# IBM/AdaMML

Measured on AMD Instinct MI355X. Metric: clips/sec (train fwd+bwd) RGB+Audio AdaMML @224^2, 5 seg, higher is better.
Workload: dtype bf16

## Files before the change

### adamml_amd/csrc/conv_gemm.hip

```cpp
#include "common.h"
#include "../../include/adamml_hip.h"
#include <type_traits>
#include <stdlib.h>
#include <stdio.h>


namespace {

constexpr int BP = 128;
constexpr int BK = 32;
constexpr int NTHREADS = 256;

struct ConvP {
    const bf16_t* x;
    const bf16_t* w;
    const float* in_scale;
    const float* in_shift;
    bf16_t* y;
    double* stats;
    int N, H, W, Cin, OH, OW, Cout, KH, KW, stride, pad, up, up_shift, act, accumulate;
    int P, K, cin_shift, n_ptiles, n_ctiles, tpb;
    size_t gx, gy;
    int in_gstride;
    const bf16_t* bn_z;
    const float* bn_vec;
    int bn_act;
    const bf16_t* res_out;
    const uint8_t* res_mask;
    int res_act;
    const bf16_t* bn_z2;
    const float* bn_vec2;
    double* stats2;
    const bf16_t* x2;
    const float* aff;
    bf16_t* side;
    const bf16_t* xb;
    int K1, C2;
    size_t gw;
    const float* epi_add;
    const float* id_scale;
    const float* id_shift;
    int id_gstride;
    uint8_t* mask_out;
    const bf16_t* pf_a;
    const float* pf_scale;
    const float* pf_shift;
    float* pf_ws;
    int pf_act, pf_gs, pf_nsplit;
    int wK;
    int cls_nt;
    unsigned cls_code;
    int oH, oW, o_ph, o_pw;
    int tp_nblk, tp_Q;
    bf16_t* tp_y;
    uint16_t* tp_code;
};

__device__ __forceinline__ int lds_off(int row, int chunk) {
    return row * 64 + ((chunk ^ (((row >> 3) & 1) << 1)) << 4);
}

template <int N, class F>
__device__ __forceinline__ void static_for(F&& f) {
    if constexpr (N > 0) {
        static_for<N - 1>(f);
        f(std::integral_constant<int, N - 1>{});
    }
}

template <int CH>
__device__ __forceinline__ int tr_swz(int row) {
    if (CH >= 128) return ((row & 3) | (((row >> 3) & 1) << 2)) << 2;
    return (((row >> 1) & 1) | (((row >> 3) & 1) << 1)) << 2;
}

__device__ const uint4 g_zero_page[4] = {};

__device__ __forceinline__ void glds16(const void* gsrc, unsigned lds_dst_uniform) {
    unsigned keep;
    asm volatile("s_mov_b32 %0, m0\n\ts_mov_b32 m0, %2\n\ts_nop 0\n\tglobal_load_lds_dwordx4 %1, off\n\ts_mov_b32 m0, %0"
                 : "=&s"(keep) : "v"(gsrc), "s"(lds_dst_uniform) : "memory");
}

constexpr int conv_gemm_wg_per_cu(int BC, int MODE, int PD, bool RES, bool DUAL, bool CAT, bool FADD, bool GLDS, int EID, int EPI) {
    if (RES || DUAL || CAT || EID) return 2;
    const int n = PD == 1 ? (BC == 128 ? 3 : 4) : (BC == 128 ? 2 : 3);
    const bool fewer = (MODE == 2 && !(BC == 128 && PD == 3)) || FADD ||
                       (BC == 64 && PD == 1 && ((EPI == 1 && !(MODE == 0 && GLDS)) || (EPI == 2 && MODE == 1))) ||
                       (BC == 128 && MODE == 1 && EPI == 2 && !GLDS);
    return fewer ? n - 1 : n;
}

template <int BC, int MODE, int PD, bool RES = false, bool DUAL = false, bool CAT = false, bool FADD = false, bool GLDS = false, int EID = 0,
          bool LZF = false, int EPI = -1, bool PF = false, int TP = 0>
__global__ __launch_bounds__(NTHREADS, conv_gemm_wg_per_cu(BC, MODE, PD, RES, DUAL, CAT, FADD, GLDS, EID, EPI)) void conv_gemm_kernel(ConvP p) {
    static_assert(TP == 0 || (FADD && EID && MODE == 0 && BC == 128 && (TP == 2 || TP == 4 || TP == 8)), "TP: FADD + EID, 128-wide cout tiles");
    constexpr int PPF = TP ? BP / TP : BP;
    constexpr int WCT = BC / 32;
    constexpr int WROWS = BC / 64;
    constexpr int TILE_BYTES = (BP + BC) * 64;
    constexpr int EPI_BYTES = BP * (BC * 2 + 16);
    constexpr int NBUF = GLDS ? 3 : 2;
    constexpr int STAGE_BYTES = (NBUF * TILE_BYTES) > EPI_BYTES ? (NBUF * TILE_BYTES) : EPI_BYTES;
    constexpr int NSR = (FADD || EPI == 0) ? 1 : 4;
    constexpr int CS_BYTES = NSR * 2 * BC * 4;
    constexpr int CS2_OFF = STAGE_BYTES + CS_BYTES + (MODE == 0 ? 0 : 256) + (MODE == 3 ? BP * 4 + 16 : 0);
    constexpr int VEC_MAXK = 1024;
    constexpr int VEC_OFF = CS2_OFF + (RES ? CS_BYTES : 0);
    constexpr int LZF_MAXK = 512;
    constexpr int PF_C = 64;
    constexpr int PF_OFF = (VEC_OFF + (LZF ? 2 * LZF_MAXK * 4 : (MODE == 0 && !GLDS) ? (DUAL ? 3 : 2) * VEC_MAXK * 4 : 0) + 1023) / 1024 * 1024;
    constexpr int SMEM_BYTES = PF ? PF_OFF + BP * PF_C * 2 : VEC_OFF + (LZF ? 2 * LZF_MAXK * 4 : (MODE == 0 && !GLDS) ? (DUAL ? 3 : 2) * VEC_MAXK * 4 : 0);
    __shared__ __attribute__((aligned(1024))) char smem[SMEM_BYTES];

    {
        const int g = blockIdx.y;
        p.x += (size_t)g * p.gx;
        p.y += (size_t)g * p.gy;
        if (p.stats) p.stats += (size_t)g * ADAMML_STAT_SLOTS * 2 * p.Cout;
        if (p.in_scale) { p.in_scale += (size_t)g * p.in_gstride; p.in_shift += (size_t)g * p.in_gstride; }
        if (p.bn_z) { p.bn_z += (size_t)g * p.gy; p.bn_vec += (size_t)g * 4 * p.Cout; }
        if (CAT) {
            p.xb += (size_t)g * (p.gx / p.K1) * p.C2;
            p.w += (size_t)g * p.gw;
            p.epi_add += (size_t)g * p.Cout;
        }
        if (DUAL) {
            p.x2 += (size_t)g * p.gx;
            p.aff += (size_t)g * 3 * p.K;
            if (p.side) p.side += (size_t)g * p.gx;
        }
        if (FADD) {
            p.bn_vec += (size_t)g * 4 * p.Cout;
            if (p.res_out) p.res_out += (size_t)g * p.gy;
            if (p.mask_out) p.mask_out += ((size_t)g * p.gy) >> 3;
            if (p.id_scale) { p.id_scale += (size_t)g * p.id_gstride; p.id_shift += (size_t)g * p.id_gstride; }
            if (TP) { p.tp_y += (size_t)g * (p.gy >> 1); if (p.tp_code) p.tp_code += ((size_t)g * (p.gy >> 1)) >> 3; }
        }
        if (PF) {
            p.pf_a += (size_t)g * p.P * PF_C;
            if (p.pf_scale) { p.pf_scale += (size_t)g * p.pf_gs; p.pf_shift += (size_t)g * p.pf_gs; }
        }
        if (RES) {
            p.res_out += (size_t)g * p.gy;
            if (p.res_mask) p.res_mask += ((size_t)g * p.gy) >> 3;
            if (p.bn_z2) { p.bn_z2 += (size_t)g * p.gy; p.bn_vec2 += (size_t)g * 4 * p.Cout; p.stats2 += (size_t)g * ADAMML_STAT_SLOTS * 2 * p.Cout; }
        }
    }
    const int tid = threadIdx.x;
    float* s_vec = reinterpret_cast<float*>(smem + (MODE == 0 ? VEC_OFF : 0));
    const int nvec = CAT ? p.C2 : p.K;
    const bool vec_lds = MODE == 0 && nvec <= VEC_MAXK && (DUAL || p.in_scale != nullptr);
    if (LZF) {
        const int kpad = (p.K + BK - 1) / BK * BK;
        for (int i = tid; i < kpad; i += NTHREADS) {
            s_vec[i] = i < p.K ? p.in_scale[i] : 0.f;
            s_vec[LZF_MAXK + i] = i < p.K ? p.in_shift[i] : 0.f;
        }
        __syncthreads();
    } else
    if (vec_lds) {
        if (DUAL) {
            for (int i = tid; i < 3 * p.K; i += NTHREADS) s_vec[i] = p.aff[i];
        } else {
            for (int i = tid; i < nvec; i += NTHREADS) { s_vec[i] = p.in_scale[i]; s_vec[nvec + i] = p.in_shift[i]; }
        }
        __syncthreads();
    }
    const int lane = tid & 63;
    const int wave = tid >> 6;
    const int wp = wave & 1;
    const int wc = wave >> 1;

    const int nwg = gridDim.x;
    int bid = blockIdx.x;
    {
        const int q = nwg >> 3, r = nwg & 7, xcd = bid & 7, idx = bid >> 3;
        bid = (xcd < r ? xcd * (q + 1) : r * (q + 1) + (xcd - r) * q) + idx;
    }
    const int ctile = bid % p.n_ctiles;
    const int pgrp = bid / p.n_ctiles;
    const int c0 = ctile * BC;

    const int chunk = tid & 3;
    const int row_a = tid >> 2;
// ... 283 lines not shown
#pragma unroll
        for (int r = 0; r < WROWS; ++r) {
            bf16x8 v = rw[SL][r];
            if (UNC && !(w_ok[r] && rkok[UNC ? SL : 0])) v = bf16x8{0, 0, 0, 0, 0, 0, 0, 0};
            *reinterpret_cast<bf16x8*>(base + BP * 64 + lds_off(row_a + r * 64, chunk)) = v;
        }
    };

    f32x4 acc[WCT][4];
#pragma unroll
    for (int i = 0; i < WCT; ++i)
#pragma unroll
        for (int j = 0; j < 4; ++j) acc[i][j] = f32x4{0.f, 0.f, 0.f, 0.f};

    const int nk = (p.K + BK - 1) / BK;
    const bool tail_rows = TP ? tp_q0 + PPF > p.tp_Q : p0 + BP > p.P;
    auto compute = [&](int buf, int kt = 0) {
        const char* base = smem + buf * TILE_BYTES;
        bf16x8 fa[4], fw[WCT];
#pragma unroll
        for (int t = 0; t < 4; ++t)
            fa[t] = *reinterpret_cast<const bf16x8*>(base + lds_off(wp * 64 + t * 16 + li, lg));
        if constexpr (LZF) {
            const f32x8 sc = load_f32x8(s_vec + kt * BK + lg * 8), sh = load_f32x8(s_vec + LZF_MAXK + kt * BK + lg * 8);
            const float lo = act_lo(p.act), hi = act_hi(p.act);
#pragma unroll
            for (int t = 0; t < 4; ++t) {
                f32x8 f = bf8_to_f32(fa[t]);
#pragma unroll
                for (int i = 0; i < 8; ++i) f[i] = clamp_act(fmaf(f[i], sc[i], sh[i]), lo, hi);
                fa[t] = f32_to_bf8(f);
            }
            if (tail_rows) {
#pragma unroll
                for (int t = 0; t < 4; ++t) {
                    const int r = wp * 64 + t * 16 + li;
                    if (TP ? tp_q0 + (r % PPF) >= p.tp_Q : p0 + r >= p.P) fa[t] = bf16x8{0, 0, 0, 0, 0, 0, 0, 0};
                }
            }
        }
#pragma unroll
        for (int t = 0; t < WCT; ++t)
            fw[t] = *reinterpret_cast<const bf16x8*>(base + BP * 64 + lds_off(wc * (BC / 2) + t * 16 + li, lg));
#pragma unroll
        for (int ct = 0; ct < WCT; ++ct)
#pragma unroll
            for (int pt = 0; pt < 4; ++pt)
                acc[ct][pt] = __builtin_amdgcn_mfma_f32_16x16x32_bf16(fw[ct], fa[pt], acc[ct][pt], 0, 0, 0);
    };
    if constexpr (GLDS) {
        const bf16_t* zeros = reinterpret_cast<const bf16_t*>(g_zero_page);
        const unsigned lds0 = (unsigned)(size_t)(__attribute__((address_space(3))) char*)smem + wave * 1024;
        const int kc8 = (chunk ^ (((row_a >> 3) & 1) << 1)) * 8;
        auto glds_stage = [&](int kt, int buf) {
            const int k = kt * BK + kc8;
            const bool kok = k < p.K;
            const unsigned base = lds0 + buf * TILE_BYTES;
            int kw_off = k;
            if (MODE == 0) {
#pragma unroll
                for (int r = 0; r < 2; ++r) {
                    const bf16_t* src = (a_ok[r] && kok) ? p.x + (size_t)(unsigned)(a_base[r] + k) : zeros;
                    glds16(src, __builtin_amdgcn_readfirstlane(base + r * 4096));
                }
            } else {
                const int tap = kok ? (k >> p.cin_shift) : 0;
                const int ci = k & (p.Cin - 1);
                const int toff = s_tapoff[tap] + ci;
                if (MODE == 3) kw_off = s_wtap[tap] + ci;
#pragma unroll
                for (int r = 0; r < 2; ++r) {
                    const bool ok = kok && ((a_mask[r] >> tap) & 1ull);
                    const bf16_t* src = ok ? p.x + (size_t)(unsigned)(a_base[r] + toff) : zeros;
                    glds16(src, __builtin_amdgcn_readfirstlane(base + r * 4096));
                }
            }
#pragma unroll
            for (int r = 0; r < WROWS; ++r) {
                const bf16_t* src = (w_ok[r] && kok) ? wrow[r] + kw_off : zeros;
                glds16(src, __builtin_amdgcn_readfirstlane(base + BP * 64 + r * 4096));
            }
        };
        constexpr int PER = 2 + WROWS;
        glds_stage(0, 0);
        if (nk > 1) glds_stage(1, 1);
        issue_eid();
        int buf = 0;
        for (int kt = 0; kt < nk; ++kt) {
            if (NEID && kt <= 1) {
                if (kt + 1 < nk) asm volatile("s_waitcnt vmcnt(%0)" ::"n"(PER + NEID) : "memory");
                else asm volatile("s_waitcnt vmcnt(%0)" ::"n"(NEID) : "memory");
            } else
            if (kt + 1 < nk) asm volatile("s_waitcnt vmcnt(%0)" ::"n"(PER) : "memory");
            else asm volatile("s_waitcnt vmcnt(0)" ::: "memory");
            __builtin_amdgcn_s_barrier();
            if (kt + 2 < nk) glds_stage(kt + 2, buf == 0 ? 2 : buf - 1);
            compute(buf, kt);
            buf = buf == 2 ? 0 : buf + 1;
        }
    } else {
    int kt0 = 0;
    if (UNC && nk >= 2 * PD) {
        static_for<PD>([&](auto sc) { issue_loads(sc, (int)decltype(sc)::value); });
        for (; kt0 + 2 * PD <= nk; kt0 += PD) {
            static_for<PD>([&](auto sc) {
                const int kt = kt0 + (int)decltype(sc)::value;
                store_tile(sc, kt & 1);
                issue_loads(sc, kt + PD);
                __syncthreads();
                compute(kt & 1);
            });
        }
    } else {
    static_for<PD>([&](auto sc) {
        if ((int)decltype(sc)::value < nk) issue_loads(sc, (int)decltype(sc)::value);
    });
    }
    issue_eid();
    for (; kt0 < nk; kt0 += PD) {
        static_for<PD>([&](auto sc) {
            const int kt = kt0 + (int)decltype(sc)::value;
            if (kt < nk) {
                store_tile(sc, kt & 1);
                if (kt + PD < nk) issue_loads(sc, kt + PD);
                __syncthreads();
                compute(kt & 1);
            }
        });
    }
    }
    __syncthreads();

    f32x8 esum, esq, esq2;
#pragma unroll
    for (int i = 0; i < 8; ++i) esum[i] = esq[i] = esq2[i] = 0.f;
#pragma unroll
    for (int pt = 0; pt < 4; ++pt)
#pragma unroll
        for (int ct = 0; ct < WCT; ++ct) {
            const int prow = wp * 64 + pt * 16 + li;
            const int ccol = wc * (BC / 2) + ct * 16 + lg * 4;
            *reinterpret_cast<bf16x4*>(smem + prow * CROW + ccol * 2) = f32_to_bf4(acc[ct][pt]);
        }
    __syncthreads();
    if (FADD) {
        if (eco < p.Cout) {
            const f32x8 sc = load_f32x8(p.bn_vec + eco), sh = load_f32x8(p.bn_vec + p.Cout + eco);
            f32x8 isc, ish;
#pragma unroll
            for (int i = 0; i < 8; ++i) { isc[i] = 1.f; ish[i] = 0.f; }
            if (p.id_scale) { isc = load_f32x8(p.id_scale + eco); ish = load_f32x8(p.id_shift + eco); }
            const float rlo = act_lo(p.res_act), rhi = act_hi(p.res_act);
            constexpr int NR = BP / RSTEP, EB = EID ? NR : (NR < 4 ? NR : 4);
            if constexpr (TP != 0) {
                static_assert(RSTEP == 16 && NR == 8, "TP epilogue mapping");
                constexpr int NPX = PPF / 16, To = TP / 2;
                bf16x8 vb[NR];
#pragma unroll
                for (int j = 0; j < NR; ++j) {
                    const int r = erow0 + j * RSTEP;
                    f32x8 f = bf8_to_f32(*reinterpret_cast<const bf16x8*>(smem + r * CROW + ech * 16));
                    const f32x8 w = bf8_to_f32(eid[j]);
#pragma unroll
                    for (int i = 0; i < 8; ++i) f[i] = clamp_act(fmaf(f[i], sc[i], sh[i]) + fmaf(w[i], isc[i], ish[i]), rlo, rhi);
                    vb[j] = f32_to_bf8(f);
                }
#pragma unroll
                for (int s = 0; s < NPX; ++s) {
                    const int q = tp_q0 + erow0 + 16 * s;
                    if (q >= p.tp_Q) continue;
#pragma unroll
                    for (int to = 0; to < To; ++to) {
                        f32x8 best;
                        unsigned code = 0;
#pragma unroll
                        for (int i = 0; i < 8; ++i) best[i] = -INFINITY;
#pragma unroll
                        for (int k = 0; k < 3; ++k) {
                            const int tt = 2 * to - 1 + k;
                            if (tt < 0 || tt >= TP) continue;
                            const f32x8 v = bf8_to_f32(vb[tt * NPX + s]);
// ... 873 lines not shown
        for (; s + 48 < nsplit; s += 64) {
            a += *reinterpret_cast<const f32x4*>(ws + (size_t)s * n + i);
            a1 += *reinterpret_cast<const f32x4*>(ws + (size_t)(s + 16) * n + i);
            a2 += *reinterpret_cast<const f32x4*>(ws + (size_t)(s + 32) * n + i);
            a3 += *reinterpret_cast<const f32x4*>(ws + (size_t)(s + 48) * n + i);
        }
        for (; s < nsplit; s += 16) a += *reinterpret_cast<const f32x4*>(ws + (size_t)s * n + i);
        a = (a + a1) + (a2 + a3);
    }
    red[ty][tx] = a;
    __syncthreads();
    if (ty == 0 && i < n) {
        f32x4 t = {0.f, 0.f, 0.f, 0.f};
#pragma unroll
        for (int k = 0; k < 16; ++k) t += red[k][tx];
        if (taps > 1) {
            const size_t per_co = (size_t)taps * cin;
#pragma unroll
            for (int q = 0; q < 4; ++q) {
                const size_t ii = i + q;
                const size_t co = ii / per_co;
                const int rem = (int)(ii - co * per_co), tap = rem / cin, ci = rem - tap * cin;
                const size_t o = (co * cin + ci) * taps + tap;
                if (store) dw[o] = t[q]; else dw[o] += t[q];
            }
        } else if ((reinterpret_cast<uintptr_t>(dw + i) & 15) == 0) {
            f32x4* o = reinterpret_cast<f32x4*>(dw + i);
            if (store) *o = t; else *o += t;
        } else {
#pragma unroll
            for (int q = 0; q < 4; ++q) { if (store) dw[i + q] = t[q]; else dw[i + q] += t[q]; }
        }
    }
}

void launch_wgrad_reduce(const float* ws, float* dw, size_t n, int nsplit, int taps, int cin, int store, int groups, hipStream_t stream) {
    if (n % 4 == 0 && (reinterpret_cast<uintptr_t>(ws) & 15) == 0)
        hipLaunchKernelGGL(wgrad_reduce4_kernel, dim3((unsigned)((n / 4 + 15) / 16), groups), dim3(256), 0, stream, ws, dw, n, nsplit, taps, cin, store);
    else
        hipLaunchKernelGGL(wgrad_reduce_kernel, dim3((unsigned)((n + 15) / 16), groups), dim3(256), 0, stream, ws, dw, n, nsplit, taps, cin, store);
}

int ilog2_exact(int v) {
    int s = 0;
    while ((1 << s) < v) ++s;
    return (1 << s) == v ? s : -1;
}

}

bool adamml_conv3x3_c64_supported(const adamml_conv_desc_t* d);
bool adamml_conv1x1_narrow_fwd_supported(const adamml_conv_desc_t* d);
bool adamml_conv1x1_narrow_wgrad_supported(const adamml_conv_desc_t* d, int cin_true);
bool adamml_conv1x1_narrow_dual_supported(const adamml_conv_desc_t* d);
bool adamml_conv1x1_narrow_dgrad_epi_supported(const adamml_conv_desc_t* d);
int adamml_conv1x1_narrow_dgrad_epi_launch(const adamml_conv_desc_t* d, const void* dz, const void* w_packed, void* dx, const void* z_in,
                                           const float* bn_vec, int act, double* sums, hipStream_t stream);
int adamml_conv1x1_narrow_dual_launch(const adamml_conv_desc_t* d, const void* g, const void* z, const float* aff, void* dz_side,
                                      const void* w_dgrad_packed, void* dx, int accumulate, const void* z_in, const float* bn_vec, int act,
                                      double* sums, hipStream_t stream);
int adamml_conv1x1_narrow_wgrad_launch(const adamml_conv_desc_t* d, const void* dz, const void* x, const float* in_scale, const float* in_shift,
                                       float* ws, int max_blocks_per_group, int* nblk_out, hipStream_t stream);
int adamml_conv1x1_narrow_fwd_launch(const adamml_conv_desc_t* d, const void* x, const void* w_packed, const float* in_scale, const float* in_shift,
                                     void* y, double* stats, hipStream_t stream);
int adamml_conv3x3_c64_launch(const adamml_conv_desc_t* d, const void* x, const void* w_packed, const float* in_scale,
                              const float* in_shift, void* y, double* stats, const void* bn_z, const float* bn_vec, int bn_act,
                              hipStream_t stream);
bool adamml_conv1x1_wide_expand_supported(const adamml_conv_desc_t* d);
int adamml_conv1x1_wide_expand_launch(const adamml_conv_desc_t* d, const void* x, const void* w_packed, const float* in_scale, const float* in_shift,
                                      void* y, double* stats, hipStream_t stream);

bool adamml_conv3x3_c64_wgrad_supported(const adamml_conv_desc_t* d, int cin_true);
int adamml_conv3x3_c64_wgrad_blocks(const adamml_conv_desc_t* d, int* tpb_out);
int adamml_conv3x3_c64_wgrad_launch(const adamml_conv_desc_t* d, const void* dz, const void* x, const float* in_scale,
                                    const float* in_shift, float* ws, hipStream_t stream);

struct DgradClass { int nt; unsigned code; int ph, pw, OHc, OWc; };
struct ResEpi { const void* res_out; const uint8_t* res_mask; int res_act; const void* bn_z2; const float* bn_vec2; double* stats2; };
struct DualIn { const void* z; const float* aff; void* side; };
struct CatIn { const void* xb; int C2; size_t gw; const float* epi_add; };
struct PfIn { const void* a; const float* scale; const float* shift; int act, gs, C; float* out; void* ws; size_t ws_bytes; };
struct FaddEpi { const float* vec; const void* idn; const float* id_scale; const float* id_shift; int id_gstride; int act; uint8_t* mask_out;
                 int tp_frames; void* tp_y; uint16_t* tp_code; };

static int conv_launch(const adamml_conv_desc_t* d, const void* x, const void* w_packed, const float* in_scale,
                       const float* in_shift, void* y, double* stats, const void* bn_z, const float* bn_vec, int bn_act,
                       hipStream_t stream, const DgradClass* cls = nullptr, const ResEpi* res = nullptr, const DualIn* dual = nullptr,
                       const CatIn* cat = nullptr, const FaddEpi* fadd = nullptr, const PfIn* pf = nullptr) {
    if (!d || !x || !w_packed || !y) return adamml_set_error(ADAMML_EINVAL, "conv_fwd: null argument");
    if (d->Cin % 8 || d->Cout % 8) return adamml_set_error(ADAMML_EINVAL, "conv_fwd: channels must be multiples of 8 (Cin=%d Cout=%d)", d->Cin, d->Cout);
    if (!cls && !fadd && adamml_conv3x3_c64_supported(d))
        return adamml_conv3x3_c64_launch(d, x, w_packed, in_scale, in_shift, y, stats, bn_z, bn_vec, bn_act, stream);
    if (!cls && !fadd && !res && !dual && !cat && !pf && !bn_z && adamml_conv1x1_narrow_fwd_supported(d))
        return adamml_conv1x1_narrow_fwd_launch(d, x, w_packed, in_scale, in_shift, y, stats, stream);
    if (!cls && !fadd && !res && !dual && !cat && !pf && !bn_z && !(d->accumulate && in_scale) && adamml_conv1x1_wide_expand_supported(d))
        return adamml_conv1x1_wide_expand_launch(d, x, w_packed, in_scale, in_shift, y, stats, stream);
    if (!cls && !fadd && !res && !dual && !cat && !pf && !in_scale && (bn_z ? stats != nullptr && !d->accumulate : d->accumulate != 0) &&
        adamml_conv1x1_narrow_dgrad_epi_supported(d))
        return adamml_conv1x1_narrow_dgrad_epi_launch(d, x, w_packed, y, bn_z, bn_vec, bn_act, stats, stream);
    ConvP p;
    p.x = (const bf16_t*)x; p.w = (const bf16_t*)w_packed; p.in_scale = in_scale; p.in_shift = in_shift;
    p.y = (bf16_t*)y; p.stats = stats;
    p.bn_z = (const bf16_t*)bn_z; p.bn_vec = bn_vec; p.bn_act = bn_act;
    p.res_out = res ? (const bf16_t*)res->res_out : nullptr; p.res_act = res ? res->res_act : 0;
    p.res_mask = res ? res->res_mask : nullptr;
    p.bn_z2 = res ? (const bf16_t*)res->bn_z2 : nullptr; p.bn_vec2 = res ? res->bn_vec2 : nullptr; p.stats2 = res ? res->stats2 : nullptr;
    p.x2 = dual ? (const bf16_t*)dual->z : nullptr; p.aff = dual ? dual->aff : nullptr; p.side = dual ? (bf16_t*)dual->side : nullptr;
    p.xb = cat ? (const bf16_t*)cat->xb : nullptr; p.K1 = d->Cin; p.C2 = cat ? cat->C2 : 0; p.gw = cat ? cat->gw : 0;
    p.epi_add = cat ? cat->epi_add : nullptr;
    p.id_scale = fadd ? fadd->id_scale : nullptr; p.id_shift = fadd ? fadd->id_shift : nullptr; p.id_gstride = fadd ? fadd->id_gstride : 0;
    p.mask_out = fadd ? fadd->mask_out : nullptr;
    p.tp_nblk = p.tp_Q = 0; p.tp_y = nullptr; p.tp_code = nullptr;
    p.pf_a = nullptr; p.pf_scale = p.pf_shift = nullptr; p.pf_ws = nullptr; p.pf_act = p.pf_gs = p.pf_nsplit = 0;
    if (fadd) { p.bn_vec = fadd->vec; p.res_out = (const bf16_t*)fadd->idn; p.res_act = fadd->act; }
    const int groups = d->groups < 1 ? 1 : d->groups;
    p.gx = (size_t)d->N * d->H * d->W * d->Cin;
    p.gy = (size_t)d->N * d->OH * d->OW * d->Cout;
    p.in_gstride = d->in_gstride;
    p.N = d->N; p.H = d->H; p.W = d->W; p.Cin = d->Cin; p.OH = d->OH; p.OW = d->OW; p.Cout = d->Cout;
    p.KH = d->KH; p.KW = d->KW; p.stride = d->stride; p.pad = d->pad; p.up = d->up < 1 ? 1 : d->up;
    p.up_shift = ilog2_exact(p.up);
    if (p.up_shift < 0) return adamml_set_error(ADAMML_EUNSUPPORTED, "conv_fwd: up=%d is not a power of two", p.up);
    p.act = d->act; p.accumulate = d->accumulate;
    p.P = d->N * d->OH * d->OW; p.K = d->KH * d->KW * d->Cin;
    if (cat) {
        if (d->KH * d->KW != 1 || d->stride != 1 || (d->up > 1) || d->Cin % BK || cat->C2 % 8 || cls || res || dual)
            return adamml_set_error(ADAMML_EUNSUPPORTED, "conv_bwd_data_alg: 1x1 / stride-1 convs with Cout %% 32 == 0 only");
        p.K = d->Cin + cat->C2;
    }
    p.wK = p.K;
    p.cls_nt = 0; p.cls_code = 0; p.oH = d->OH; p.oW = d->OW; p.o_ph = p.o_pw = 0;
    if (cls) {
        p.cls_nt = cls->nt; p.cls_code = cls->code; p.o_ph = cls->ph; p.o_pw = cls->pw;
        p.OH = cls->OHc; p.OW = cls->OWc;
        p.P = d->N * cls->OHc * cls->OWc;
        p.K = cls->nt * d->Cin;
    }
    const bool multitap = d->KH * d->KW > 1 || cls;
    p.cin_shift = 0;
    if (multitap) {
        p.cin_shift = ilog2_exact(d->Cin);
        if (p.cin_shift < 0) return adamml_set_error(ADAMML_EUNSUPPORTED, "conv_fwd: KxK conv needs power-of-two Cin (got %d)", d->Cin);
    }
    if (p.P <= 0) return ADAMML_OK;
    bool narrow = d->Cout <= 64 || (d->Cout % 128 != 0 && d->Cout < 256);
    if (!narrow && (long)ceil_div(p.P, BP) * ceil_div(d->Cout, 128) * groups < 512) narrow = true;
    const int tp = fadd ? fadd->tp_frames : 0;
    if (tp) narrow = false;
    const int BC = narrow ? 64 : 128;
    p.n_ptiles = ceil_div(p.P, BP);
    if (tp) {
        p.tp_Q = d->OH * d->OW;
        p.tp_nblk = ceil_div(p.tp_Q, BP / tp);
        p.n_ptiles = (d->N / tp) * p.tp_nblk;
        p.tp_y = (bf16_t*)fadd->tp_y; p.tp_code = fadd->tp_code;
    }
    p.n_ctiles = ceil_div(d->Cout, BC);
    p.tpb = (int)((long)p.n_ptiles * p.n_ctiles * groups / 2048);
    if (p.tpb < 1) p.tpb = 1;
    if (p.tpb > 8) p.tpb = 8;
    if (pf) {
        const long target = 1536;
        long nsp = target / ((long)p.n_ctiles * groups);
        if (nsp < 1) nsp = 1;
        p.tpb = (int)ceil_div(p.n_ptiles, (int)nsp);
        if (p.tpb < 1) p.tpb = 1;
    }
    dim3 grid(ceil_div(p.n_ptiles, p.tpb) * p.n_ctiles, groups), block(NTHREADS);
    const int taps = d->KH * d->KW;
    if ((long)d->N * d->H * d->W * d->Cin >= (1L << 31)) return adamml_set_error(ADAMML_EUNSUPPORTED, "conv_fwd: input tensor exceeds 2^31 elements");
    const int mode = cls ? 3 : (p.up > 1 ? 2 : (multitap ? (taps <= 64 ? 1 : 2) : 0));
    if (mode == 2 && !multitap) { p.cin_shift = 30; }
    const int nk = ceil_div(p.K, BK);
    const bool deep = (long)grid.x * grid.y <= 768 && nk >= 8 && mode != 1;
    if (fadd) {
        if (mode != 0 || res || dual || cat || stats) return adamml_set_error(ADAMML_EUNSUPPORTED, "conv_fwd_bn_add: only 1x1 / stride-1 convs");
        if (!in_scale || p.K <= 512) {
            const bool eid = p.res_out != nullptr;
            if (tp) {
#define LAUNCH_TP(TV)                                                                                                                                        \
                do {                                                                                                                                         \
                    if (in_scale) hipLaunchKernelGGL((conv_gemm_kernel<128, 0, 1, false, false, false, true, true, 1, true, -1, false, TV>), grid, block, 0, stream, p);  \
                    else hipLaunchKernelGGL((conv_gemm_kernel<128, 0, 1, false, false, false, true, true, 1, false, -1, false, TV>), grid, block, 0, stream, p);         \
                } while (0)
                if (tp == 8) LAUNCH_TP(8); else if (tp == 4) LAUNCH_TP(4); else LAUNCH_TP(2);
#undef LAUNCH_TP
                return adamml_check_launch("conv_fwd_bn_add_tpool");
            }
#define LAUNCH_FADD(BCV)                                                                                                                   \
            do {                                                                                                                           \
                if (in_scale) {                                                                                                            \
                    if (eid) hipLaunchKernelGGL((conv_gemm_kernel<BCV, 0, 1, false, false, false, true, true, 1, true>), grid, block, 0, stream, p);  \
                    else hipLaunchKernelGGL((conv_gemm_kernel<BCV, 0, 1, false, false, false, true, true, 0, true>), grid, block, 0, stream, p);      \
                } else {                                                                                                                   \
                    if (eid) hipLaunchKernelGGL((conv_gemm_kernel<BCV, 0, 1, false, false, false, true, true, 1, false>), grid, block, 0, stream, p); \
                    else hipLaunchKernelGGL((conv_gemm_kernel<BCV, 0, 1, false, false, false, true, true, 0, false>), grid, block, 0, stream, p);     \
                }                                                                                                                          \
            } while (0)
            if (BC == 64) LAUNCH_FADD(64); else LAUNCH_FADD(128);
#undef LAUNCH_FADD
        } else
        if (tp) return adamml_set_error(ADAMML_EUNSUPPORTED, "conv_fwd_bn_add_tpool: needs the LDS-DMA kernel (K <= 512 for a lazy input)");
        else
        if (BC == 64) hipLaunchKernelGGL((conv_gemm_kernel<64, 0, 1, false, false, false, true>), grid, block, 0, stream, p);
        else hipLaunchKernelGGL((conv_gemm_kernel<128, 0, 1, false, false, false, true>), grid, block, 0, stream, p);
        return adamml_check_launch("conv_fwd_bn_add");
    }
    if (res) {
        if (mode != 0) return adamml_set_error(ADAMML_EUNSUPPORTED, "conv_bwd_data_res: only 1x1 / stride-1 convs");
        if (pf) {
            if (BC != 128 || d->Cout % 128 || pf->C != 64 || in_scale || !p.res_mask || !p.accumulate || p.bn_z || p.bn_z2 || !stats)
                return adamml_set_error(ADAMML_EUNSUPPORTED, "conv_bwd_data_res_prod: needs Cout %% 128 == 0, a 64-channel product operand, "
                                                             "the accumulate + 1-bit-mask + sum(g')-only form");
            p.pf_nsplit = ceil_div(p.n_ptiles, p.tpb);
            const size_t need = (size_t)groups * p.n_ctiles * p.pf_nsplit * 128 * 64 * sizeof(float);
            if (!pf->ws || pf->ws_bytes < need) return adamml_set_error(ADAMML_EINVAL, "conv_bwd_data_res_prod: workspace too small (need %zu bytes)", need);
            p.pf_a = (const bf16_t*)pf->a; p.pf_scale = pf->scale; p.pf_shift = pf->scale ? pf->shift : nullptr; p.pf_act = pf->act; p.pf_gs = pf->gs;
            p.pf_ws = (float*)pf->ws;
            hipLaunchKernelGGL((conv_gemm_kernel<128, 0, 1, true, false, false, false, true, 1, false, -1, true>), grid, block, 0, stream, p);
            int rc = adamml_check_launch("conv_bwd_data_res_prod");
            if (rc) return rc;
            launch_wgrad_reduce((const float*)pf->ws, pf->out, (size_t)128 * 64, p.pf_nsplit, 1, 64, 1, groups * p.n_ctiles, stream);
            return adamml_check_launch("conv_bwd_data_res_prod (reduce)");
        }
        if (in_scale) return adamml_set_error(ADAMML_EUNSUPPORTED, "conv_bwd_data_res: the gradient operand is never lazy");
        if (p.res_mask && p.accumulate && !p.bn_z && !p.bn_z2) {
            if (BC == 64) hipLaunchKernelGGL((conv_gemm_kernel<64, 0, 1, true, false, false, false, true, 1>), grid, block, 0, stream, p);
            else hipLaunchKernelGGL((conv_gemm_kernel<128, 0, 1, true, false, false, false, true, 1>), grid, block, 0, stream, p);
        } else {
            if (BC == 64) hipLaunchKernelGGL((conv_gemm_kernel<64, 0, 1, true, false, false, false, true>), grid, block, 0, stream, p);
            else hipLaunchKernelGGL((conv_gemm_kernel<128, 0, 1, true, false, false, false, true>), grid, block, 0, stream, p);
        }
        return adamml_check_launch("conv_bwd_data_res");
    }
    if (cat) {
        if (mode != 0) return adamml_set_error(ADAMML_EUNSUPPORTED, "conv_bwd_data_alg: only 1x1 / stride-1 convs");
        if (BC == 64) hipLaunchKernelGGL((conv_gemm_kernel<64, 0, 3, false, false, true>), grid, block, 0, stream, p);
        else hipLaunchKernelGGL((conv_gemm_kernel<128, 0, 3, false, false, true>), grid, block, 0, stream, p);
        return adamml_check_launch("conv_bwd_data_alg");
    }
    if (dual) {
        if (mode != 0 || res) return adamml_set_error(ADAMML_EUNSUPPORTED, "conv_bwd_data_dual: only 1x1 / stride-1 convs");
        if (BC == 64) hipLaunchKernelGGL((conv_gemm_kernel<64, 0, 3, false, true>), grid, block, 0, stream, p);
        else hipLaunchKernelGGL((conv_gemm_kernel<128, 0, 2, false, true>), grid, block, 0, stream, p);
        return adamml_check_launch("conv_bwd_data_dual");
    }
    const bool glds = !in_scale && mode != 2;
    const int epi = bn_z ? 1 : (p.accumulate ? 2 : 0);
#define LAUNCH_EPI(BCV, MODEV, GL)                                                                                                          \
    do {                                                                                                                                    \
        if (epi == 0) hipLaunchKernelGGL((conv_gemm_kernel<BCV, MODEV, 1, false, false, false, false, GL, 0, false, 0>), grid, block, 0, stream, p);       \
        else if (epi == 1) hipLaunchKernelGGL((conv_gemm_kernel<BCV, MODEV, 1, false, false, false, false, GL, 0, false, 1>), grid, block, 0, stream, p);  \
        else hipLaunchKernelGGL((conv_gemm_kernel<BCV, MODEV, 1, false, false, false, false, GL, 0, false, 2>), grid, block, 0, stream, p);               \
    } while (0)
#define LAUNCH_CONV(BCV, MODEV)                                                                             \
    do {                                                                                                    \
        if (glds) LAUNCH_EPI(BCV, MODEV, true);                                                             \
        else if (deep) hipLaunchKernelGGL((conv_gemm_kernel<BCV, MODEV, 3>), grid, block, 0, stream, p);     \
        else LAUNCH_EPI(BCV, MODEV, false);                                                                 \
    } while (0)
    if (BC == 64) {
        if (mode == 0) LAUNCH_CONV(64, 0); else if (mode == 1) LAUNCH_CONV(64, 1);
        else if (mode == 2) { if (deep) hipLaunchKernelGGL((conv_gemm_kernel<64, 2, 3>), grid, block, 0, stream, p); else hipLaunchKernelGGL((conv_gemm_kernel<64, 2, 1>), grid, block, 0, stream, p); }
        else if (glds) LAUNCH_EPI(64, 3, true);
        else LAUNCH_EPI(64, 3, false);
    } else {
        if (mode == 0) LAUNCH_CONV(128, 0); else if (mode == 1) LAUNCH_CONV(128, 1);
        else if (mode == 2) { if (deep) hipLaunchKernelGGL((conv_gemm_kernel<128, 2, 3>), grid, block, 0, stream, p); else hipLaunchKernelGGL((conv_gemm_kernel<128, 2, 1>), grid, block, 0, stream, p); }
        else if (glds) LAUNCH_EPI(128, 3, true);
        else LAUNCH_EPI(128, 3, false);
    }
#undef LAUNCH_CONV
#undef LAUNCH_EPI
    return adamml_check_launch("conv_fwd");
}

extern "C" int adamml_conv1x1_narrow_supported(const adamml_conv_desc_t* d, int kind) {
    if (!d) return 0;
    if (kind == 0) return adamml_conv1x1_narrow_fwd_supported(d) ? 1 : 0;
    if (kind == 1) return adamml_conv1x1_narrow_wgrad_supported(d, d->Cin) ? 1 : 0;
    if (kind == 2) return adamml_conv1x1_narrow_dual_supported(d) ? 1 : 0;
    adamml_conv_desc_t g = *d;
    g.H = d->OH; g.W = d->OW; g.Cin = d->Cout; g.OH = d->H; g.OW = d->W; g.Cout = d->Cin; g.accumulate = 0;
    if (kind == 3) return adamml_conv1x1_narrow_fwd_supported(&g) ? 1 : 0;
    if (kind == 4) return adamml_conv1x1_narrow_dgrad_epi_supported(&g) ? 1 : 0;
    return 0;
}

extern "C" int adamml_conv1x1_wide_supported(const adamml_conv_desc_t* d, int kind) {
    if (!d) return 0;
    if (kind == 0) { adamml_conv_desc_t f = *d; f.accumulate = 0; return adamml_conv1x1_wide_expand_supported(&f) ? 1 : 0; }
    if (kind != 3 && kind != 4) return 0;
    if (d->stride != 1) return 0;
    adamml_conv_desc_t g = *d;
    g.H = d->OH; g.W = d->OW; g.Cin = d->Cout; g.OH = d->H; g.OW = d->W; g.Cout = d->Cin; g.accumulate = kind == 4; g.up = 1; g.pad = 0;
    return adamml_conv1x1_wide_expand_supported(&g) ? 1 : 0;
}

extern "C" int adamml_conv_fused_input_supported(const adamml_conv_desc_t* d) {
    return d && adamml_conv3x3_c64_supported(d) ? 1 : 0;
}

extern "C" int adamml_conv_fwd(const adamml_conv_desc_t* d, const void* x, const void* w_packed, const float* in_scale,
                               const float* in_shift, void* y, double* stats, hipStream_t stream) {
    return conv_launch(d, x, w_packed, in_scale, in_shift, y, stats, nullptr, nullptr, 0, stream);
}

extern "C" int adamml_conv_fwd_bn_add_supported(const adamml_conv_desc_t* d) {
    return d && d->KH == 1 && d->KW == 1 && d->stride == 1 && d->pad == 0 && (d->up <= 1) && d->Cin % 8 == 0 && d->Cout % 8 == 0 ? 1 : 0;
}

int adamml_conv1x1_fadd_stream_supported(const adamml_conv_desc_t* d);
int adamml_conv1x1_fadd_stream_launch(const adamml_conv_desc_t* d, const void* x, const void* w_packed, const float* in_scale, const float* in_shift,
                                      const float* bn_vec, const void* idn, const float* id_scale, const float* id_shift, int id_gstride, int act,
                                      void* out, uint8_t* mask_out, hipStream_t stream);
extern "C" int adamml_conv_fwd_bn_add_streams(const adamml_conv_desc_t* d) {
    return d && adamml_conv_fwd_bn_add_supported(d) && adamml_conv1x1_fadd_stream_supported(d) ? 1 : 0;
}

extern "C" int adamml_conv_fwd_bn_add(const adamml_conv_desc_t* d, const void* x, const void* w_packed, const float* in_scale,
                                      const float* in_shift, const float* bn_vec, const void* idn, const float* id_scale,
                                      const float* id_shift, int id_gstride, int act, void* out, uint8_t* mask_out, hipStream_t stream) {
    if (!adamml_conv_fwd_bn_add_supported(d)) return adamml_set_error(ADAMML_EUNSUPPORTED, "conv_fwd_bn_add: 1x1 / stride-1 convs only");
    if (!bn_vec) return adamml_set_error(ADAMML_EINVAL, "conv_fwd_bn_add: null BatchNorm vectors");
    if (idn && adamml_conv1x1_fadd_stream_supported(d))
        return adamml_conv1x1_fadd_stream_launch(d, x, w_packed, in_scale, in_shift, bn_vec, idn, id_scale, id_shift, id_gstride, act, out, mask_out, stream);
    FaddEpi f{bn_vec, idn, id_scale, id_shift, id_gstride, act, mask_out, 0, nullptr, nullptr};
    return conv_launch(d, x, w_packed, in_scale, in_shift, out, nullptr, nullptr, nullptr, 0, stream, nullptr, nullptr, nullptr, nullptr, &f);
}

bool adamml_conv1x1_fadd_next_supported(const adamml_conv_desc_t* d, int next_cout);
int adamml_conv1x1_fadd_next_launch(const adamml_conv_desc_t* d, const void* x, const void* w_packed, const float* in_scale, const float* in_shift,
                                    const float* bn_vec, const void* idn, const float* id_scale, const float* id_shift, int id_gstride, int act,
                                    void* out, uint8_t* mask_out, const void* w1_packed, void* y1, double* stats1, hipStream_t stream);

extern "C" int adamml_conv_fwd_bn_add_next_supported(const adamml_conv_desc_t* d, int next_cout) {
    return d && next_cout > 0 && adamml_conv_fwd_bn_add_supported(d) && adamml_conv1x1_fadd_next_supported(d, next_cout) ? 1 : 0;
}

extern "C" int adamml_conv_fwd_bn_add_next(const adamml_conv_desc_t* d, const void* x, const void* w_packed, const float* in_scale,
                                           const float* in_shift, const float* bn_vec, const void* idn, const float* id_scale,
                                           const float* id_shift, int id_gstride, int act, void* out, uint8_t* mask_out, const void* w_next,
                                           void* y_next, double* stats_next, hipStream_t stream) {
    if (!d || !x || !w_packed || !bn_vec || !out || !w_next || !y_next) return adamml_set_error(ADAMML_EINVAL, "conv_fwd_bn_add_next: null argument");
    if (!adamml_conv_fwd_bn_add_next_supported(d, 64))
        return adamml_set_error(ADAMML_EUNSUPPORTED, "conv_fwd_bn_add_next: 1x1 / stride-1, 64 -> 256 channels, next conv 256 -> 64 only");
    return adamml_conv1x1_fadd_next_launch(d, x, w_packed, in_scale, in_shift, bn_vec, idn, id_scale, id_shift, id_gstride, act, out, mask_out,
                                           w_next, y_next, stats_next, stream);
}

bool adamml_conv1x1_fadd_tpool_supported(const adamml_conv_desc_t* d, int frames);
int adamml_conv1x1_fadd_tpool_launch(const adamml_conv_desc_t* d, const void* x, const void* w_packed, const float* in_scale, const float* in_shift,
                                     const float* bn_vec, const void* idn, const float* id_scale, const float* id_shift, int id_gstride, int act,
                                     int frames, void* pooled, uint16_t* code, hipStream_t stream);

int adamml_conv1x1_fadd_tpool_stream_supported(const adamml_conv_desc_t* d, int frames);
// ... 534 lines not shown
```

### include/adamml_hip.h

```cpp
#ifndef ADAMML_HIP_H
#define ADAMML_HIP_H
#include <stddef.h>
#include <stdint.h>
#ifdef __cplusplus
extern "C" {
#endif

typedef struct ihipStream_t* hipStream_t;
typedef struct ihipEvent_t* hipEvent_t;

#define ADAMML_API __attribute__((visibility("default")))

#define ADAMML_STAT_SLOTS 32

#define ADAMML_ACT_NONE 0
#define ADAMML_ACT_RELU 1
#define ADAMML_ACT_RELU6 2

typedef struct {
    int32_t N, H, W, Cin;
    int32_t OH, OW, Cout;
    int32_t KH, KW, stride, pad;
    int32_t up;
    int32_t act;
    int32_t accumulate;
    int32_t groups;
    int32_t in_gstride;
} adamml_conv_desc_t;

ADAMML_API int adamml_version(void);
ADAMML_API const char* adamml_last_error_string(void);
ADAMML_API int adamml_set_deterministic(int on);
ADAMML_API int adamml_get_deterministic(void);

ADAMML_API int adamml_conv_fwd(const adamml_conv_desc_t* d, const void* x, const void* w_packed, const float* in_scale,
                    const float* in_shift, void* y, double* stats, hipStream_t stream);
ADAMML_API int adamml_conv_fused_input_supported(const adamml_conv_desc_t* d);
ADAMML_API int adamml_conv1x1_narrow_supported(const adamml_conv_desc_t* d, int kind);
ADAMML_API int adamml_conv1x1_wide_supported(const adamml_conv_desc_t* d, int kind);
ADAMML_API int adamml_conv_fwd_bn_add_supported(const adamml_conv_desc_t* d);
ADAMML_API int adamml_conv_fwd_bn_add_streams(const adamml_conv_desc_t* d);
ADAMML_API int adamml_conv_fwd_bn_add(const adamml_conv_desc_t* d, const void* x, const void* w_packed, const float* in_scale, const float* in_shift,
                           const float* bn_vec, const void* idn, const float* id_scale, const float* id_shift, int id_gstride, int act,
                           void* out, uint8_t* mask_out, hipStream_t stream);
ADAMML_API int adamml_conv_fwd_bn_add_next_supported(const adamml_conv_desc_t* d, int next_cout);
ADAMML_API int adamml_conv_fwd_bn_add_next(const adamml_conv_desc_t* d, const void* x, const void* w_packed, const float* in_scale, const float* in_shift,
                                const float* bn_vec, const void* idn, const float* id_scale, const float* id_shift, int id_gstride, int act,
                                void* out, uint8_t* mask_out, const void* w_next, void* y_next, double* stats_next, hipStream_t stream);
ADAMML_API int adamml_conv_fwd_bn_add_tpool_supported(const adamml_conv_desc_t* d, int frames, int act, int lazy_input);
ADAMML_API int adamml_conv_fwd_bn_add_tpool_streams(const adamml_conv_desc_t* d, int frames);
ADAMML_API int adamml_conv_fwd_bn_add_tpool(const adamml_conv_desc_t* d, const void* x, const void* w_packed, const float* in_scale, const float* in_shift,
                                 const float* bn_vec, const void* idn, const float* id_scale, const float* id_shift, int id_gstride, int act,
                                 int frames, void* pooled, uint16_t* code, hipStream_t stream);
ADAMML_API int adamml_gram_stats(const void* w_packed, const float* G, const float* s, double* sums, int Cout, int Cin, int groups, hipStream_t stream);
ADAMML_API int adamml_gram_colsum_supported(int C);
ADAMML_API size_t adamml_gram_colsum_workspace(size_t P, int C, int groups);
ADAMML_API int adamml_gram_colsum(const void* x, const float* scale, const float* shift, int gstride, int act, float* G, float* s, size_t P, int C,
                       int groups, void* workspace, size_t workspace_bytes, hipStream_t stream);
ADAMML_API int adamml_conv_bwd_data(const adamml_conv_desc_t* d, const void* dz, const void* w_dgrad_packed, void* dx,
                         int accumulate, hipStream_t stream);
ADAMML_API int adamml_conv_bwd_data_bn(const adamml_conv_desc_t* d, const void* dz, const void* w_dgrad_packed, void* dx, const void* z_in,
                            const float* bn_vec, int act, double* sums, hipStream_t stream);

ADAMML_API int adamml_conv_bwd_data_dual_supported(const adamml_conv_desc_t* d);
ADAMML_API int adamml_bn_bwd_affine(const float* coef, const float* vec, float* aff, int C, int groups, hipStream_t stream);
ADAMML_API int adamml_conv_bwd_data_dual(const adamml_conv_desc_t* d, const void* g, const void* z, const float* aff, void* dz_side,
                              const void* w_dgrad_packed, void* dx, int accumulate, const void* z_in, const float* bn_vec, int act,
                              double* sums, hipStream_t stream);

ADAMML_API int adamml_conv_bwd_weight_grouped(const adamml_conv_desc_t* d, const void* dz, const float* dz_scale, const float* dz_shift, int dz_act,
                                   int dz_gstride, const void* x, const float* in_scale, const float* in_shift, float* out, int cin_true,
                                   void* workspace, size_t workspace_bytes, hipStream_t stream);
ADAMML_API int adamml_lazy_colsum(const void* x, const float* scale, const float* shift, int gstride, int act, float* s, size_t P, int C, int groups,
                       hipStream_t stream);
ADAMML_API int adamml_alg_sumfix(const float* w, const float* P, const float* vec, double* sums, int Cout, int Cin, int groups, hipStream_t stream);
ADAMML_API int adamml_alg_pack(const float* w, const float* aff, const float* m_pre, void* w_alg, float* epi_add, int Cout, int Cin, int groups,
                    hipStream_t stream);
ADAMML_API int adamml_alg_wgrad_combine(const float* w, const float* aff, const float* P, const float* G, const float* wg_pre, const float* s, float* dw,
                             int Cout, int Cin, int groups, hipStream_t stream);
ADAMML_API int adamml_conv_bwd_data_alg(const adamml_conv_desc_t* d, const void* g, const void* a, const float* a_scale, const float* a_shift,
                             const void* w_alg, const float* epi_add, void* dx, int accumulate, const void* z_in, const float* bn_vec,
                             int act, double* sums, hipStream_t stream);

ADAMML_API int adamml_conv_bwd_data_res_supported(const adamml_conv_desc_t* d);
ADAMML_API int adamml_conv_bwd_data_res_streams(const adamml_conv_desc_t* d);
ADAMML_API int adamml_conv_bwd_data_res(const adamml_conv_desc_t* d, const void* dz, const void* w_dgrad_packed, void* dx,
                             int accumulate, const void* res_out, const uint8_t* res_mask, int res_act, const void* z_a, const float* vec_a,
                             double* sums_a, const void* z_b, const float* vec_b, double* sums_b, hipStream_t stream);

ADAMML_API int adamml_conv_bwd_data_res_prod_supported(const adamml_conv_desc_t* d, int a_channels);
ADAMML_API size_t adamml_conv_bwd_data_res_prod_workspace(const adamml_conv_desc_t* d);
ADAMML_API int adamml_conv_bwd_data_res_prod_streams(const adamml_conv_desc_t* d, int a_channels);
ADAMML_API int adamml_conv_bwd_data_res_prod(const adamml_conv_desc_t* d, const void* dz, const void* w_dgrad_packed, void* dx, const uint8_t* res_mask,
                                  int res_act, double* sums_a, const void* a, const float* a_scale, const float* a_shift, int a_act,
                                  int a_gstride, int a_channels, float* prod, void* workspace, size_t workspace_bytes, hipStream_t stream);

ADAMML_API size_t adamml_conv_bwd_weight_workspace(const adamml_conv_desc_t* d, int cin_true);
ADAMML_API int adamml_conv_bwd_weight(const adamml_conv_desc_t* d, const void* dz, const void* x, const float* in_scale,
                           const float* in_shift, float* dw, int cin_true, void* workspace, size_t workspace_bytes,
                           hipStream_t stream);
ADAMML_API int adamml_pack_conv_weight(const float* w, void* out, int cout, int cin_true, int cin_pad, int kh, int kw, int mode,
                            hipStream_t stream);

ADAMML_API int adamml_conv_stem_supported(const adamml_conv_desc_t* d);
ADAMML_API int adamml_pack_stem_weight(const float* w, void* out, int cout, int cin_true, hipStream_t stream);
ADAMML_API int adamml_conv_stem_fwd(const adamml_conv_desc_t* d, const void* x, const void* w_stem_packed, void* y, double* stats,
                         hipStream_t stream);
ADAMML_API size_t adamml_conv_stem_bwd_weight_workspace(const adamml_conv_desc_t* d);
ADAMML_API int adamml_conv_stem_bwd_weight(const adamml_conv_desc_t* d, const void* dz, const void* x, float* dw, int cin_true,
                                void* workspace, size_t workspace_bytes, hipStream_t stream);

ADAMML_API int adamml_dwconv_fwd(const adamml_conv_desc_t* d, const void* x, const float* w_tapmajor, const float* in_scale,
                      const float* in_shift, void* y, double* stats, hipStream_t stream);
ADAMML_API int adamml_dwconv_bwd_data(const adamml_conv_desc_t* d, const void* dz, const float* w_tapmajor, void* dx,
                           int accumulate, hipStream_t stream);
ADAMML_API int adamml_dwconv_bwd_data_bn_supported(const adamml_conv_desc_t* d);
ADAMML_API int adamml_dwconv_bwd_data_bn(const adamml_conv_desc_t* d, const void* dz, const float* w_tapmajor, void* dx, const void* z_in,
                              const float* bn_vec, int act, double* sums, hipStream_t stream);
ADAMML_API size_t adamml_dwconv_bwd_weight_workspace(const adamml_conv_desc_t* d);
ADAMML_API int adamml_dwconv_bwd_fused_supported(const adamml_conv_desc_t* d);
ADAMML_API size_t adamml_dwconv_bwd_fused_workspace(const adamml_conv_desc_t* d);
ADAMML_API int adamml_dwconv_bwd_fused(const adamml_conv_desc_t* d, const void* g, const void* z, const float* aff, const float* w_tapmajor,
                            const void* x, const float* x_vec, int x_act, void* dx, double* sums, float* dw, void* workspace,
                            size_t workspace_bytes, hipStream_t stream);
ADAMML_API int adamml_conv_stem1_supported(const adamml_conv_desc_t* d);
ADAMML_API int adamml_conv_stem1_fwd(const adamml_conv_desc_t* d, const float* x, size_t image_stride, size_t group_stride, const float* w_tapmajor,
                          void* y, double* stats, hipStream_t stream);
ADAMML_API size_t adamml_conv_stem1_bwd_weight_workspace(const adamml_conv_desc_t* d);
ADAMML_API int adamml_conv_stem1_bwd_weight(const adamml_conv_desc_t* d, const void* dz, const float* x, size_t image_stride, size_t group_stride,
                                 float* dw , void* workspace,
                                 size_t workspace_bytes, hipStream_t stream);
ADAMML_API int adamml_dwconv_bwd_weight(const adamml_conv_desc_t* d, const void* dz, const void* x, const float* in_scale,
                             const float* in_shift, float* dw, void* workspace, size_t workspace_bytes, hipStream_t stream);

ADAMML_API int adamml_stats_collapse(const double* stats, double* out, int C, int groups, hipStream_t stream);
ADAMML_API int adamml_bn_finalize(const double* stats, int nslots, int groups, double count, const float* gamma, const float* beta,
                       float* running_mean, float* running_var, float momentum, float eps, float* bn_vec, int C,
                       hipStream_t stream);
ADAMML_API int adamml_bn_eval_affine(const float* gamma, const float* beta, const float* running_mean, const float* running_var,
                          float eps, float* scale, float* shift, int C, hipStream_t stream);
ADAMML_API int adamml_bn_act_add(const void* z, const float* scale, const float* shift, int z_gstride, int act, const void* idn,
                      const float* id_scale, const float* id_shift, int id_gstride, void* out, size_t P, int C, int groups,
                      hipStream_t stream);
ADAMML_API int adamml_bn_act_add_mask(const void* z, const float* scale, const float* shift, int z_gstride, int act, const void* idn,
                           const float* id_scale, const float* id_shift, int id_gstride, void* out, uint8_t* mask_out, size_t P,
                           int C, int groups, hipStream_t stream);
ADAMML_API int adamml_act_bwd_from_output(const void* g_out, const void* out, int act, void* g, size_t n, hipStream_t stream);
ADAMML_API int adamml_residual_bwd(const void* g_out, const void* out, int act, void* g2, const void* za, const float* veca, double* sumsa,
                        const void* zb, const float* vecb, double* sumsb, size_t P, int C, int groups, hipStream_t stream);
ADAMML_API int adamml_bn_bwd_reduce(const void* g, const void* z, const float* bn_vec, int act, double* sums, size_t P, int C, int groups,
                         hipStream_t stream);
ADAMML_API int adamml_bn_bwd_finalize(const double* sums, int nslots, int groups, double count, const float* gamma, const float* bn_vec,
                           float* dgamma, float* dbeta, float* coef, int C, float grad_scale, hipStream_t stream);
ADAMML_API int adamml_bn_bwd_finalize_affine(const double* sums, int nslots, int groups, double count, const float* gamma, const float* bn_vec,
                                  float* dgamma, float* dbeta, float* coef, float* aff, int C, float grad_scale, hipStream_t stream);
ADAMML_API int adamml_bn_bwd_apply(const void* g, const void* z, const float* bn_vec, int act, const float* coef, void* dz, size_t P, int C,
                        int groups, hipStream_t stream);

ADAMML_API int adamml_maxpool2d_fwd(const void* x, const float* scale, const float* shift, int gstride, int act, void* y, uint8_t* idx,
                         void* z_sel, int N, int H, int W, int C, int OH, int OW, int groups, hipStream_t stream);
ADAMML_API int adamml_maxpool2d_bwd(const void* g_y, const uint8_t* idx, void* g_x, int N, int H, int W, int C, int OH, int OW,
                         int accumulate, hipStream_t stream);
ADAMML_API int adamml_temporal_pool_fwd(const void* x, const float* scale, const float* shift, int gstride, int act, void* y, int NB,
                             int T, size_t HWC, int C, int mode, int groups, hipStream_t stream);
ADAMML_API int adamml_temporal_pool_bwd(const void* g_y, const void* x, const float* scale, const float* shift, int gstride, int act,
                             void* g_x, int NB, int T, size_t HWC, int C, int mode, int groups, hipStream_t stream);
ADAMML_API int adamml_maxpool2d_bwd_bn_reduce(const void* g_y, const uint8_t* idx, const void* z, const float* vec, int act, double* sums,
                                   int N, int H, int W, int C, int OH, int OW, int groups, hipStream_t stream);
ADAMML_API int adamml_maxpool2d_bwd_bn_apply(const void* g_y, const uint8_t* idx, const void* z, const float* vec, int act, const float* coef,
                                  void* dz, int N, int H, int W, int C, int OH, int OW, int groups, hipStream_t stream);

ADAMML_API int adamml_temporal_pool_bwd_res_supported(int T, int C, int mode);
ADAMML_API int adamml_temporal_pool_bwd_res(const void* g_y, const void* out, int act, void* g2, const void* z_a, const float* vec_a,
                                 double* sums_a, int NB, int T, int HW, int C, int groups, hipStream_t stream);
ADAMML_API int adamml_temporal_pool_bwd_code(const void* g_y, const uint16_t* code, void* g2, double* sums_a, int NB, int T, int HW, int C, int groups,
                                  hipStream_t stream);
ADAMML_API int adamml_temporal_pool_bwd_code_prod_supported(int T, int C, int Cin);
ADAMML_API size_t adamml_temporal_pool_bwd_code_prod_workspace(int NB, int T, int HW, int C, int Cin, int groups);
ADAMML_API int adamml_temporal_pool_bwd_code_prod(const void* g_y, const uint16_t* code, void* g2, double* sums_a, const void* a, const float* in_scale,
                                       const float* in_shift, int in_gstride, int in_act, float* prod, void* workspace, size_t workspace_bytes,
                                       int NB, int T, int HW, int C, int Cin, int groups, hipStream_t stream);

ADAMML_API int adamml_gap_fwd(const void* x, const float* scale, const float* shift, int gstride, int act, float* out, int N, int HW,
// ... 79 lines not shown
```

Measured before the change: 3429.

## Add two-K-tile-per-stage LDS-DMA pipeline variant for 128-wide conv GEMM

Adds a K2 template variant of the LDS-DMA conv GEMM that fetches two K tiles per stage into four LDS buffers and synchronises once per pair, halving waitcnt and barrier count per K step. A shape heuristic picks it by default for mode-3 convs with wide input or deep K. It also adds a runtime policy override and launch counters. The trade-off is a larger LDS footprint with occupancy capped at two workgroups per CU, plus a full vmcnt(0) drain each stage instead of a rolling wait.

```diff
diff --git a/adamml_amd/csrc/conv_gemm.hip b/adamml_amd/csrc/conv_gemm.hip
--- a/adamml_amd/csrc/conv_gemm.hip
+++ b/adamml_amd/csrc/conv_gemm.hip
@@ -1,6 +1,7 @@
 #include "common.h"
 #include "../../include/adamml_hip.h"
 #include <type_traits>
+#include <atomic>
 #include <stdlib.h>
 #include <stdio.h>
 
@@ -82,7 +83,8 @@
                  : "=&s"(keep) : "v"(gsrc), "s"(lds_dst_uniform) : "memory");
 }
 
-constexpr int conv_gemm_wg_per_cu(int BC, int MODE, int PD, bool RES, bool DUAL, bool CAT, bool FADD, bool GLDS, int EID, int EPI) {
+constexpr int conv_gemm_wg_per_cu(int BC, int MODE, int PD, bool RES, bool DUAL, bool CAT, bool FADD, bool GLDS, int EID, int EPI, bool K2 = false) {
+    if (K2) return 2;
     if (RES || DUAL || CAT || EID) return 2;
     const int n = PD == 1 ? (BC == 128 ? 3 : 4) : (BC == 128 ? 2 : 3);
     const bool fewer = (MODE == 2 && !(BC == 128 && PD == 3)) || FADD ||
@@ -92,15 +94,16 @@
 }
 
 template <int BC, int MODE, int PD, bool RES = false, bool DUAL = false, bool CAT = false, bool FADD = false, bool GLDS = false, int EID = 0,
-          bool LZF = false, int EPI = -1, bool PF = false, int TP = 0>
-__global__ __launch_bounds__(NTHREADS, conv_gemm_wg_per_cu(BC, MODE, PD, RES, DUAL, CAT, FADD, GLDS, EID, EPI)) void conv_gemm_kernel(ConvP p) {
+          bool LZF = false, int EPI = -1, bool PF = false, int TP = 0, bool K2 = false>
+__global__ __launch_bounds__(NTHREADS, conv_gemm_wg_per_cu(BC, MODE, PD, RES, DUAL, CAT, FADD, GLDS, EID, EPI, K2)) void conv_gemm_kernel(ConvP p) {
+    static_assert(!K2 || (GLDS && PD == 1 && BC == 128 && !EID && !PF && !LZF), "K2: the plain 128-wide LDS-DMA instances");
     static_assert(TP == 0 || (FADD && EID && MODE == 0 && BC == 128 && (TP == 2 || TP == 4 || TP == 8)), "TP: FADD + EID, 128-wide cout tiles");
     constexpr int PPF = TP ? BP / TP : BP;
     constexpr int WCT = BC / 32;
     constexpr int WROWS = BC / 64;
     constexpr int TILE_BYTES = (BP + BC) * 64;
     constexpr int EPI_BYTES = BP * (BC * 2 + 16);
-    constexpr int NBUF = GLDS ? 3 : 2;
+    constexpr int NBUF = K2 ? 4 : (GLDS ? 3 : 2);
     constexpr int STAGE_BYTES = (NBUF * TILE_BYTES) > EPI_BYTES ? (NBUF * TILE_BYTES) : EPI_BYTES;
     constexpr int NSR = (FADD || EPI == 0) ? 1 : 4;
     constexpr int CS_BYTES = NSR * 2 * BC * 4;
@@ -550,6 +553,23 @@
             }
         };
         constexpr int PER = 2 + WROWS;
+        if constexpr (K2) {
+            const int ns = (nk + 1) >> 1;
+            auto stage2 = [&](int s, int sb) {
+                glds_stage(2 * s, 2 * sb);
+                glds_stage(2 * s + 1, 2 * sb + 1);
+            };
+            stage2(0, 0);
+            int sb = 0;
+            for (int s = 0; s < ns; ++s) {
+                asm volatile("s_waitcnt vmcnt(0)" ::: "memory");
+                __builtin_amdgcn_s_barrier();
+                if (s + 1 < ns) stage2(s + 1, sb ^ 1);
+                compute(2 * sb, 2 * s);
+                if (2 * s + 1 < nk) compute(2 * sb + 1, 2 * s + 1);
+                sb ^= 1;
+            }
+        } else {
         glds_stage(0, 0);
         if (nk > 1) glds_stage(1, 1);
         issue_eid();
@@ -565,6 +585,7 @@
             if (kt + 2 < nk) glds_stage(kt + 2, buf == 0 ? 2 : buf - 1);
             compute(buf, kt);
             buf = buf == 2 ? 0 : buf + 1;
+        }
         }
     } else {
     int kt0 = 0;
@@ -1604,6 +1625,27 @@
 struct PfIn { const void* a; const float* scale; const float* shift; int act, gs, C; float* out; void* ws; size_t ws_bytes; };
 struct FaddEpi { const float* vec; const void* idn; const float* id_scale; const float* id_shift; int id_gstride; int act; uint8_t* mask_out;
                  int tp_frames; void* tp_y; uint16_t* tp_code; };
+
+static std::atomic<long long> g_kstage_counts[2];
+static std::atomic<int> g_kstage_policy{0};
+
+static bool conv_kstage(int mode, int nk, int cls_nt, int cin) {
+    const int policy = g_kstage_policy.load(std::memory_order_relaxed);
+    if (policy) return policy == 1;
+    return mode == 3 && ((cls_nt >= 2 && cin >= 256) || nk >= 64);
+}
+
+extern "C" int adamml_conv_kstage_counts(long long* out2) {
+    if (!out2) return adamml_set_error(ADAMML_EINVAL, "conv_kstage_counts: null argument");
+    for (int i = 0; i < 2; ++i) out2[i] = g_kstage_counts[i].load(std::memory_order_relaxed);
+    return ADAMML_OK;
+}
+
+extern "C" int adamml_conv_kstage_policy(int policy) {
+    if (policy < 0 || policy > 2) return adamml_set_error(ADAMML_EINVAL, "conv_kstage_policy: 0 = by shape, 1 = wherever compiled, 2 = never");
+    g_kstage_policy.store(policy, std::memory_order_relaxed);
+    return ADAMML_OK;
+}
 
 static int conv_launch(const adamml_conv_desc_t* d, const void* x, const void* w_packed, const float* in_scale,
                        const float* in_shift, void* y, double* stats, const void* bn_z, const float* bn_vec, int bn_act,
@@ -1769,12 +1811,15 @@
     }
     const bool glds = !in_scale && mode != 2;
     const int epi = bn_z ? 1 : (p.accumulate ? 2 : 0);
-#define LAUNCH_EPI(BCV, MODEV, GL)                                                                                                          \
+    const bool k2 = glds && BC == 128 && conv_kstage(mode, nk, p.cls_nt, d->Cin);
+    g_kstage_counts[k2 ? 0 : 1].fetch_add(1, std::memory_order_relaxed);
+#define LAUNCH_EPI_K(BCV, MODEV, GL, KV)                                                                                                     \
     do {                                                                                                                                    \
-        if (epi == 0) hipLaunchKernelGGL((conv_gemm_kernel<BCV, MODEV, 1, false, false, false, false, GL, 0, false, 0>), grid, block, 0, stream, p);       \
-        else if (epi == 1) hipLaunchKernelGGL((conv_gemm_kernel<BCV, MODEV, 1, false, false, false, false, GL, 0, false, 1>), grid, block, 0, stream, p);  \
-        else hipLaunchKernelGGL((conv_gemm_kernel<BCV, MODEV, 1, false, false, false, false, GL, 0, false, 2>), grid, block, 0, stream, p);               \
+        if (epi == 0) hipLaunchKernelGGL((conv_gemm_kernel<BCV, MODEV, 1, false, false, false, false, GL, 0, false, 0, false, 0, KV>), grid, block, 0, stream, p);       \
+        else if (epi == 1) hipLaunchKernelGGL((conv_gemm_kernel<BCV, MODEV, 1, false, false, false, false, GL, 0, false, 1, false, 0, KV>), grid, block, 0, stream, p);  \
+        else hipLaunchKernelGGL((conv_gemm_kernel<BCV, MODEV, 1, false, false, false, false, GL, 0, false, 2, false, 0, KV>), grid, block, 0, stream, p);               \
     } while (0)
+#define LAUNCH_EPI(BCV, MODEV, GL) LAUNCH_EPI_K(BCV, MODEV, GL, false)
 #define LAUNCH_CONV(BCV, MODEV)                                                                             \
     do {                                                                                                    \
         if (glds) LAUNCH_EPI(BCV, MODEV, true);                                                             \
@@ -1787,6 +1832,8 @@
         else if (glds) LAUNCH_EPI(64, 3, true);
         else LAUNCH_EPI(64, 3, false);
     } else {
+        if (k2) { if (mode == 0) LAUNCH_EPI_K(128, 0, true, true); else if (mode == 1) LAUNCH_EPI_K(128, 1, true, true); else LAUNCH_EPI_K(128, 3, true, true); }
+        else
         if (mode == 0) LAUNCH_CONV(128, 0); else if (mode == 1) LAUNCH_CONV(128, 1);
         else if (mode == 2) { if (deep) hipLaunchKernelGGL((conv_gemm_kernel<128, 2, 3>), grid, block, 0, stream, p); else hipLaunchKernelGGL((conv_gemm_kernel<128, 2, 1>), grid, block, 0, stream, p); }
         else if (glds) LAUNCH_EPI(128, 3, true);
@@ -1794,6 +1841,7 @@
     }
 #undef LAUNCH_CONV
 #undef LAUNCH_EPI
+#undef LAUNCH_EPI_K
     return adamml_check_launch("conv_fwd");
 }
 
diff --git a/include/adamml_hip.h b/include/adamml_hip.h
--- a/include/adamml_hip.h
+++ b/include/adamml_hip.h
@@ -99,6 +99,8 @@
 ADAMML_API int adamml_conv_bwd_weight(const adamml_conv_desc_t* d, const void* dz, const void* x, const float* in_scale,
                            const float* in_shift, float* dw, int cin_true, void* workspace, size_t workspace_bytes,
                            hipStream_t stream);
+ADAMML_API int adamml_conv_kstage_counts(long long* out2);
+ADAMML_API int adamml_conv_kstage_policy(int policy);
 ADAMML_API int adamml_pack_conv_weight(const float* w, void* out, int cout, int cin_true, int cin_pad, int kh, int kw, int mode,
                             hipStream_t stream);
 
```

After: 3428. About the same (-0.0%).
